# tiborcamargo/KinectPy

Measured on NVIDIA B200. Metric: fused_3kinect_frames_per_s, higher is better.
Workload: dtype f64

## Files before the change

### kinectpy_b200/csrc/kp_batch.cuh

```cuda
#pragma once
#include "kp_common.cuh"
#include "kp_grid.cuh"
#include "kp_vbi.cuh"

struct DCnt {
    const int32_t *p;
    int stride;
#ifdef __CUDACC__
    __device__ __forceinline__ int at(int s) const { return p[(size_t)s * stride]; }
#endif
};
struct DOut {
    int32_t *p;
    int stride;
#ifdef __CUDACC__
    __device__ __forceinline__ int32_t &at(int s) const { return p[(size_t)s * stride]; }
#endif
};
static inline DCnt dcnt(const int32_t *p, size_t stride_bytes) { return DCnt{p, (int)(stride_bytes / 4)}; }
static inline DOut dout(int32_t *p, size_t stride_bytes) { return DOut{p, (int)(stride_bytes / 4)}; }

struct KpVoxDev {
    double minb[3];
    double voxel;
// ... 1 lines not shown
    unsigned int sentinel;
    int imax[3];
    int ok;
};

struct BLaunch {
    kp_ctx *ctx;
    int nseg;
    int64_t cap;
    int ctas;
};

constexpr int BC_THREADS = 256;
constexpr int BC_ITEMS = 8;
constexpr int BC_TILE = BC_THREADS * BC_ITEMS;

struct BScan {
    int32_t *tile_sum;
    unsigned int *ticket;
    int max_tiles;
};

int kp_b_compact_rows(const BLaunch &L, const BScan &S, DCnt n, const uint8_t *mask, int64_t mask_stride, int invert,
                      const float *in, float *out, int64_t row_stride, DOut total, const uint32_t *aux_in = nullptr,
                      uint32_t *aux_out = nullptr);
int kp_b_partition_rows(const BLaunch &L, const BScan &S, DCnt n, const uint8_t *mask, int64_t mask_stride, const float *in,
                        float *out_true, float *out_false, int64_t row_stride, DOut total, const uint32_t *aux_in = nullptr,
                        uint32_t *aux_true = nullptr, uint32_t *aux_false = nullptr);
int kp_b_compact_index(const BLaunch &L, const BScan &S, DCnt n, const uint8_t *mask, int64_t mask_stride, int32_t *list,
                       int64_t list_stride, DOut total);
int kp_b_run_starts_u32(const BLaunch &L, const BScan &S, DCnt n, const uint32_t *keys, int64_t key_stride, int32_t *run_start,
                        int64_t rs_stride, DOut total);
int kp_b_exclusive_scan(const BLaunch &L, const BScan &S, DCnt n, int32_t *v, int64_t v_stride, DOut total);

struct BSort {
    int32_t *g_hist;
    int32_t *g_tot;
};
int kp_b_sort_pairs_u32(const BLaunch &L, const BSort &W, int64_t n, int passes, uint32_t *keys, uint32_t *keys_tmp,
                        int32_t *vals, int32_t *vals_tmp, int64_t stride);
size_t kp_b_sort_hist_elems(int64_t n);

int kp_b_csum(const BLaunch &L, DCnt n, const double *x, int64_t x_stride, int mode, const double *aux, int64_t aux_stride,
              double *tmp, int64_t tmp_stride, double *out, int64_t out_stride);

struct KpKnnSegDesc {
    const KpGridDev *g0, *g1;
    const KpVbiDev *vbi;
    const float4 *pts0;
    const int32_t *n;
    uint8_t *flags0, *flags1;
    int32_t *list0, *list1;
    const int32_t *cnt0, *cnt1;
    const KpGridDev *gm;
    uint8_t *flags_m; int32_t *list_m; const int32_t *cnt_m;
    double *mean;
    const float *cloud;
    float *normals;
};
struct KpKnnBatch {
    void *d_params = nullptr, *h_params = nullptr;
    int nseg = 0, k = 0, mode = 0, cap_hist = 0, cap_warp = 0, rad = 1, cap_mid = 0, has_mid = 0;
};
int kp_knn_batch_create(kp_ctx *ctx, const KpKnnSegDesc *segs, int nseg, int k, int mode, double radius, double rho_a, double rho_b,
                        KpKnnBatch *out);
int kp_knn_batch_vbi(kp_ctx *ctx, const KpKnnBatch &b, int64_t cap_rows);
void kp_knn_batch_destroy(KpKnnBatch *b);
int kp_knn_batch_level0(kp_ctx *ctx, const KpKnnBatch &b, int64_t cap_rows);
int kp_knn_batch_mid(kp_ctx *ctx, const KpKnnBatch &b, int64_t cap_rows);
int kp_knn_batch_level1(kp_ctx *ctx, const KpKnnBatch &b, int64_t cap_rows);
int kp_knn_batch_stragglers(kp_ctx *ctx, const KpKnnBatch &b);

struct KpIcpPairDesc {
    const KpGridDev *tgt_grid;
    const KpVbiDev *tgt_vbi;
    const float *tgt_normals;
    const float *src;
    const int32_t *n_src;
    double init_T[16];
    double *res_T, *res_fit, *res_rmse; int32_t *res_iters;
};
struct KpIcpBatch {
    void *d_params = nullptr, *d_work = nullptr;
    int npairs = 0, max_iter = 0, grid = 0;
    int64_t cap_src = 0;
};
int kp_icp_batch_create(kp_ctx *ctx, const KpIcpPairDesc *pairs, int npairs, int64_t cap_src, double max_corr, int max_iter,
                        double rel_fitness, double rel_rmse, KpIcpBatch *out);
void kp_icp_batch_destroy(KpIcpBatch *b);
int kp_icp_batch_run(kp_ctx *ctx, const KpIcpBatch &b);
```

### kinectpy_b200/csrc/kp_engine.cu

```cuda
#include <stdlib.h>
#include <string.h>
#include <string>
#include <vector>
#include "kp_batch.cuh"

int kp_unproject_engine(kp_ctx *ctx, const uint16_t *d_depth, const float *d_xytab, const double *h_T, int B, int S, int64_t P,
                        int flags, double scale, float *d_xyz, float *d_xyz_raw, int32_t *d_slots, int32_t *d_rows,
                        const uint8_t *d_rgb, const double *d_crop_med, double crop_gate);
size_t kp_unproject_engine_slots(int B, int S, int64_t P);
int kp_crop_median_engine(kp_ctx *ctx, const uint16_t *d_depth, const uint32_t *d_vbits, int B, int S, int64_t P, uint32_t *d_hist,
                          double *d_med);
size_t kp_crop_median_hist_elems();
int kp_resample_engine(kp_ctx *ctx, const float *const *d_base, int64_t stride, const int32_t *d_n, int64_t n_step, int B, int64_t N, int mode,
                       uint64_t seed, const int64_t *h_ids, int32_t *d_status, int64_t status_step, uint32_t *keys, uint32_t *hist,
                       void *st, unsigned long long *list, float *d_out);
size_t kp_resample_engine_hist_elems();
size_t kp_resample_engine_state_bytes();
int64_t kp_resample_engine_cap(int64_t N);
bool kp_resample_engine_fits(int64_t N);

namespace {
constexpr int ENG_MAX_S = 6;
constexpr int ENG_MAX_CAND = 16;

// ... 2041 lines not shown
    return KP_OK;
}

int kp_pipeline_destroy(kp_pipeline *p)
{
    if (!p) return KP_OK;
    cudaSetDevice(p->device);
    for (auto &s : p->slots) slot_destroy(s);
    if (p->d_tab) cudaFree(p->d_tab);
    if (p->d_vbits) cudaFree(p->d_vbits);
    if (p->h_res) cudaFreeHost(p->h_res);
    delete p;
    return KP_OK;
}

const char *kp_pipeline_last_error(kp_pipeline *p) { return p ? p->err.c_str() : kp_last_error(nullptr); }

int kp_pipeline_run(kp_pipeline *p, const uint16_t *depth, int depth_on_device, int64_t F, kp_frame_result *h_results,
                    float *d_out_xyz, int64_t out_stride)
{
    return run_impl(p, depth, nullptr, depth_on_device, F, nullptr, h_results, d_out_xyz, out_stride, nullptr);
}

int kp_pipeline_run_ex(kp_pipeline *p, const uint16_t *depth, const uint8_t *rgb, int inputs_on_device, int64_t F,
                       const int64_t *h_frame_ids, kp_frame_result *h_results, float *d_out_xyz, int64_t out_stride, float *d_fixed)
{
    return run_impl(p, depth, rgb, inputs_on_device, F, h_frame_ids, h_results, d_out_xyz, out_stride, d_fixed);
}

int kp_pipeline_run_host(kp_pipeline *p, const uint16_t *h_depth, int64_t F, kp_frame_result *h_results, float *h_out_xyz,
                         int64_t out_stride)
{
    if (p && h_out_xyz) {
        cudaPointerAttributes at;
        if (cudaPointerGetAttributes(&at, h_out_xyz) != cudaSuccess || (at.type != cudaMemoryTypeHost && at.type != cudaMemoryTypeManaged)) {
            cudaGetLastError();
            p->err = "kp_pipeline_run_host: h_out_xyz must be pinned host memory (kp_host_alloc)";
            return KP_E_ARG;
        }
    }
    return run_impl(p, h_depth, nullptr, 0, F, nullptr, h_results, h_out_xyz, out_stride, nullptr);
}

int64_t kp_pipeline_launch_count(kp_pipeline *p)
{
    int64_t n = 0;
    if (p) {
        n = p->launches;
        for (auto &s : p->slots) n += s.ctx->launches + s.aux->launches;
    }
    return n;
}

int kp_pipeline_frames_in_flight(kp_pipeline *p, int *batch, int *slots)
{
    if (!p) return KP_E_ARG;
    if (batch) *batch = p->B;
    if (slots) *slots = p->W;
    return KP_OK;
}

int kp_pipeline_frame_counts(kp_pipeline *p, int64_t *h_counts, int n)
{
    if (!p || !h_counts || n < 26) return KP_E_ARG;
    cudaSetDevice(p->device);
    EngSlot &s = p->slots[0];
    if (cudaStreamSynchronize(s.ctx->stream) != cudaSuccess) return KP_E_CUDA;
    EngDyn d;
    if (cudaMemcpy(&d, s.dyn, sizeof d, cudaMemcpyDeviceToHost) != cudaSuccess) return KP_E_CUDA;
    std::vector<EngCloud> cl((size_t)p->cfg.S);
    if (cudaMemcpy(cl.data(), s.icl, sizeof(EngCloud) * cl.size(), cudaMemcpyDeviceToHost) != cudaSuccess) return KP_E_CUDA;
    const int64_t v[8] = {d.n_fused, d.n_voxel, d.n_sor, d.n_lo, d.n_rest, d.n_merged, d.n_fsor, d.n_out};
    for (int i = 0; i < 8; ++i) h_counts[i] = v[i];
    for (int i = 0; i < 3; ++i) { h_counts[8 + i] = d.cnt_l0[i]; h_counts[11 + i] = d.cnt_l1[i]; }
    for (int i = 0; i < 6; ++i) { h_counts[14 + i] = i < p->cfg.S ? cl[i].nv : 0; h_counts[20 + i] = i < p->cfg.S ? cl[i].n : 0; }
    if (n >= 29)
        for (int i = 0; i < 3; ++i) h_counts[26 + i] = d.cnt_lm[i];
    if (n >= 35) {
        double med[ENG_MAX_S] = {0.0};
        if (p->cfg.do_crop && cudaMemcpy(med, s.crop_med, sizeof(double) * p->cfg.S, cudaMemcpyDeviceToHost) != cudaSuccess) return KP_E_CUDA;
        for (int i = 0; i < 6; ++i) h_counts[29 + i] = i < p->cfg.S ? (int64_t)(2.0 * med[i]) : 0;
    }
    if (n >= 36) h_counts[35] = p->cfg.ror_nb_points > 0 ? d.n_ror : 0;
    return KP_OK;
}

int kp_pipeline_profile(kp_pipeline *p, int enable_or_read, int max_entries, const char **h_names, double *h_ms,
                        int64_t *h_calls, double *h_bytes, int *h_n)
{
    if (!p) return KP_E_ARG;
    cudaSetDevice(p->device);
    kp_ctx *ctx = p->slots[0].ctx;
    if (enable_or_read == 1 || enable_or_read == 0) {
        kp_profile_reset(ctx);
        kp_profile_enable(ctx, enable_or_read);
        p->profiling = enable_or_read == 1;
        return KP_OK;
    }
    return kp_profile_read(ctx, max_entries, h_names, h_ms, h_calls, h_bytes, h_n);
}

}
```

### kinectpy_b200/csrc/kp_icp.cu

```cuda
#include <math.h>
#include <string.h>
#include <stdlib.h>
#include <vector>
#include "kp_grid.cuh"
#include "kp_batch.cuh"
#include "kp_umeyama.cuh"

namespace {
#ifndef ICP_THREADS_N
#define ICP_THREADS_N 256
#endif
constexpr int ICP_THREADS = ICP_THREADS_N;
#ifndef ICP_MIN_CTAS
#define ICP_MIN_CTAS 4
#endif
constexpr int ICP_GROUP = 32;
constexpr int ICP_NV = 29;
enum { ICP_PLANE = 0, ICP_POINT = 1, ICP_COLORED = 2 };

struct IcpState {
    double T[16];
    double U[16];
    double fitness, rmse;
    long long ncorr;
    int done, iters;
    unsigned int ticket;
    int pass;
    double slack;
};

struct IcpParams {
    KpGridDev g;
    const float *tgt_normals;
    int mode;
    const float *src_int;
    const float *tgt_int;
    const float *tgt_grad;
    double sqrt_lg, sqrt_lp;
    double *cur;
    int32_t *corr;
    int ns;
    double r2;
    double slack;
    int max_iter;
    double rel_fit, rel_rmse;
    IcpState *st;
    double *slots;
    double *gslots;
    unsigned int *gticket;
    const KpGridDev *gdev;
    const int32_t *ns_dev;
    const float *src;
    double max_corr;
    double init_T[16];
    double *res_T, *res_fit, *res_rmse; int32_t *res_iters;
    const KpVbiDev *vbi;
};

__device__ __forceinline__ double icp_slack(const KpGridDev &g, double max_corr)
{
    double M = 0.0;
    for (int c = 0; c < 3; ++c)
        M = fmax(M, fmax(fabs(g.org[c]), fabs(g.org[c] + g.cell * (double)g.dim[c])) + 2.0 * max_corr);
    const double eps = 8.0 * M / 16777216.0;
    return eps * (2.0 * max_corr + eps) * 1.000001 + 4e-6 * (max_corr * max_corr);
}

__device__ __forceinline__ IcpParams icp_params_batched(const IcpParams *__restrict__ pp)
{
    IcpParams p = pp[blockIdx.y];
    p.g = *p.gdev;
    p.ns = *p.ns_dev;
    p.slack = p.st->slack;
    return p;
}

__global__ void __launch_bounds__(256) k_icp_init(const float *src, int ns, const __grid_constant__ IcpParams p, IcpState init,
                                                  double *out)
{
    int i = blockIdx.x * blockDim.x + threadIdx.x;
    if (i == 0) *p.st = init;
    if (i >= ns) return;
    const double *T = init.T;
    double X = src[3 * (int64_t)i], Y = src[3 * (int64_t)i + 1], Z = src[3 * (int64_t)i + 2];
    out[3 * (int64_t)i] = kp_affine(T[0], T[1], T[2], T[3], X, Y, Z);
    out[3 * (int64_t)i + 1] = kp_affine(T[4], T[5], T[6], T[7], X, Y, Z);
    out[3 * (int64_t)i + 2] = kp_affine(T[8], T[9], T[10], T[11], X, Y, Z);
}

__device__ __forceinline__ int icp_nearest(const KpGridDev &g, double sx, double sy, double sz, double r2, double slack, int prev)
{
    int bpos = -1;
    const int cx = kp_cell_coord(g, sx, 0), cy = kp_cell_coord(g, sy, 1), cz = kp_cell_coord(g, sz, 2);
    double bd = INFINITY;
    int bi = -1;
    const float fx32 = (float)sx, fy32 = (float)sy, fz32 = (float)sz;
    if (prev >= 0) {
        const float4 q = __ldg(g.pts + prev);
        const double d2 = kp_d2(sx, sy, sz, (double)q.x, (double)q.y, (double)q.z);
        if (d2 < r2) { bd = d2; bi = __float_as_int(q.w); bpos = prev; }
    }
    float flo[3], fhi[3];
    {
        const double cs = g.cell * (1.0 - 3.0 / 1048576.0);
        const double ss[3] = {sx, sy, sz};
        const int cc[3] = {cx, cy, cz};
#pragma unroll
        for (int c = 0; c < 3; ++c) {
            const double f = fmin(fmax((ss[c] - g.org[c]) * g.inv_cell - (double)cc[c], 0.0), 1.0);
            flo[c] = (float)(f * cs); fhi[c] = (float)((1.0 - f) * cs);
        }
    }
    const double lim0 = fmin(bd, r2);
    const float budget = __double2float_ru(lim0 * (1.0 + 4e-6));
    int2 rng[9];
#pragma unroll
    for (int oi = 0; oi < 9; ++oi) {
        const int dx = oi / 3 - 1, dy = oi % 3 - 1;
        const float gx = dx < 0 ? flo[0] : (dx > 0 ? fhi[0] : 0.0f), gy = dy < 0 ? flo[1] : (dy > 0 ? fhi[1] : 0.0f);
        const float zb = budget - (gx * gx + gy * gy);
        const int zlo = flo[2] * flo[2] <= zb ? cz - 1 : cz, zhi = fhi[2] * fhi[2] <= zb ? cz + 1 : cz;
        rng[oi] = zb >= 0.0f ? kp_span_range(g, cx + dx, cy + dy, zlo, zhi) : make_int2(0, 0);
    }
    float lim32 = __double2float_ru(lim0 + slack), cur = budget;
    const int order[9] = {4, 1, 3, 5, 7, 0, 2, 6, 8};
#pragma unroll
    for (int k = 0; k < 9; ++k) {
        const int oi = order[k], dx = oi / 3 - 1, dy = oi % 3 - 1;
        const float gx = dx < 0 ? flo[0] : (dx > 0 ? fhi[0] : 0.0f), gy = dy < 0 ? flo[1] : (dy > 0 ? fhi[1] : 0.0f);
        if (gx * gx + gy * gy > cur) continue;
        for (int t = rng[oi].x; t < rng[oi].y; t += 4) {
            const int m = rng[oi].y - t;
            float4 q[4];
            q[0] = __ldg(g.pts + t);
            q[1] = __ldg(g.pts + (m > 1 ? t + 1 : t));
            q[2] = __ldg(g.pts + (m > 2 ? t + 2 : t));
            q[3] = __ldg(g.pts + (m > 3 ? t + 3 : t));
            float d32[4];
#pragma unroll
            for (int u = 0; u < 4; ++u) {
                const float ex = fx32 - q[u].x, ey = fy32 - q[u].y, ez = fz32 - q[u].z;
                d32[u] = __fmaf_rn(ez, ez, __fmaf_rn(ey, ey, ex * ex));
            }
#pragma unroll
            for (int u = 0; u < 4; ++u) {
                if (u >= m || d32[u] > lim32) continue;
                const double d2 = kp_d2(sx, sy, sz, (double)q[u].x, (double)q[u].y, (double)q[u].z);
                const int id = __float_as_int(q[u].w);
                if (d2 < r2 && (d2 < bd || (d2 == bd && id < bi))) {
                    bd = d2; bi = id; bpos = t + u;
                    lim32 = __double2float_ru(bd + slack); cur = __double2float_ru(bd * (1.0 + 4e-6));
                }
            }
        }
    }
    return bpos;
}

__device__ __forceinline__ int icp_nearest_vbi(const KpVbiDev &v, double sx, double sy, double sz, double r2, double slack, int prev)
{
    int bpos = -1, bi = -1;
    double bd = INFINITY;
    if (prev >= 0) {
        const float4 q = __ldg(v.pts + prev);
        const double d2 = kp_d2(sx, sy, sz, (double)q.x, (double)q.y, (double)q.z);
        if (d2 < r2) { bd = d2; bi = __float_as_int(q.w); bpos = prev; }
    }
    const double lim0 = fmin(bd, r2);
    const double rad = sqrt(lim0) * (1.0 + 1e-6) + v.eps + v.voxel * 1e-6;
    KpVbiBox box;
    if (!kp_vbi_box(v, sx, sy, sz, rad, box)) return bpos;
    const float fx32 = (float)sx, fy32 = (float)sy, fz32 = (float)sz;
    float lim32 = __double2float_ru(lim0 + slack);
    kp_vbi_visit(v, box, [&](int pos, const float4 &q) {
        const float ex = fx32 - q.x, ey = fy32 - q.y, ez = fz32 - q.z;
        const float d32 = __fmaf_rn(ez, ez, __fmaf_rn(ey, ey, ex * ex));
        if (d32 > lim32) return;
        const double d2 = kp_d2(sx, sy, sz, (double)q.x, (double)q.y, (double)q.z);
        const int id = __float_as_int(q.w);
        if (d2 < r2 && (d2 < bd || (d2 == bd && id < bi))) {
            bd = d2; bi = id; bpos = pos;
            lim32 = __double2float_ru(bd + slack);
        }
    });
    return bpos;
}

__device__ bool icp_solve6_cta(double (*M)[7], double *x, int tid)
{
    const int r = tid / 7, j = tid % 7;
    const bool own = tid < 42;
    bool ok = true;
    for (int c = 0; c < 6; ++c) {
        int pv = c;
        double best = fabs(M[c][c]);
        for (int rr = c + 1; rr < 6; ++rr) {
            const double v = fabs(M[rr][c]);
            if (v > best) { best = v; pv = rr; }
        }
        if (!(best > 1e-300)) { ok = false; break; }
        __syncthreads();
        if (own && r == c && pv != c) { const double t = M[c][j]; M[c][j] = M[pv][j]; M[pv][j] = t; }
        __syncthreads();
        double nv = 0.0;
        const bool upd = own && r > c && j >= c;
        if (upd) { const double f = M[r][c] / M[c][c]; nv = M[r][j] - f * M[c][j]; }
        __syncthreads();
        if (upd) M[r][j] = nv;
        __syncthreads();
    }
    if (ok && tid == 0) {
        for (int rr = 5; rr >= 0; --rr) {
            double sacc = M[rr][6];
            for (int jj = rr + 1; jj < 6; ++jj) sacc -= M[rr][jj] * x[jj];
            x[rr] = sacc / M[rr][rr];
        }
    }
    __syncthreads();
    if (ok)
        for (int rr = 0; rr < 6; ++rr) if (!isfinite(x[rr])) ok = false;
    return ok;
}

__device__ void icp_finish(const IcpParams &p, IcpState *st, const double *tot, int pass, int tid)
{
    __shared__ double M[6][7];
    __shared__ double x[6];
    __shared__ double Un[16];
    __shared__ int s_done;
    const double nc = tot[28];
    if (tid == 0) {
        const double fit = p.ns > 0 ? nc / (double)p.ns : 0.0;
        const double rmse = nc > 0 ? sqrt(tot[27] / nc) : 0.0;
        const double pfit = st->fitness, prmse = st->rmse;
        st->fitness = fit; st->rmse = rmse; st->ncorr = (long long)nc;
        st->ticket = 0;
        st->pass = pass + 1;
        bool done = false;
        if (pass > 0) {
            st->iters = pass;
            if (fabs(pfit - fit) < p.rel_fit && fabs(prmse - rmse) < p.rel_rmse) done = true;
        }
        if (pass >= p.max_iter) done = true;
        if (done) st->done = 1;
        s_done = done ? 1 : 0;
    }
    if (tid < 16) Un[tid] = (tid % 5 == 0) ? 1.0 : 0.0;
    if (tid < 6) x[tid] = 0.0;
    __syncthreads();
    if (s_done) return;
    if (p.mode == ICP_POINT) {
        if (tid == 0 && nc > 0) kp_umeyama(tot, nc, Un);
    } else {
        if (tid < 42) {
            const int r = tid / 7, j = tid % 7;
            if (j == 6) M[r][6] = -tot[21 + r];
            else {
                const int a = r < j ? r : j, b = r < j ? j : r;
                M[r][j] = tot[a * 6 - (a * (a - 1)) / 2 + (b - a)];
            }
        }
        __syncthreads();
        const bool ok = icp_solve6_cta(M, x, tid);
        if (ok && nc > 0 && tid == 0) {
            double ca = cos(x[0]), sa = sin(x[0]), cb = cos(x[1]), sb = sin(x[1]), cg = cos(x[2]), sg = sin(x[2]);
            Un[0] = cg * cb; Un[1] = cg * sb * sa - sg * ca; Un[2] = cg * sb * ca + sg * sa; Un[3] = x[3];
            Un[4] = sg * cb; Un[5] = sg * sb * sa + cg * ca; Un[6] = sg * sb * ca - cg * sa; Un[7] = x[4];
            Un[8] = -sb;     Un[9] = cb * sa;                Un[10] = cb * ca;               Un[11] = x[5];
        }
    }
    __syncthreads();
    double tn = 0.0;
    if (tid < 16) {
        const int i2 = tid >> 2, j = tid & 3;
        for (int k = 0; k < 4; ++k) tn = tn + Un[4 * i2 + k] * st->T[4 * k + j];
    }
    __syncthreads();
    if (tid < 16) { st->T[tid] = tn; st->U[tid] = Un[tid]; }
    __threadfence();
}

template <int MODE>
__device__ __forceinline__ void icp_iter_body(const IcpParams &p)
{
    __shared__ double sh[ICP_THREADS / 32][ICP_NV];
    __shared__ double part[ICP_THREADS / 32][32];
    __shared__ double tot[ICP_NV];
    __shared__ unsigned int s_ticket;
    IcpState *st = p.st;
    const int tid = threadIdx.x, lane = tid & 31, warp = tid >> 5;
    const int i = blockIdx.x * ICP_THREADS + tid;
    double sx0 = 0.0, sy0 = 0.0, sz0 = 0.0;
    int prev0 = -1;
    if (i < p.ns) {
        sx0 = p.cur[3 * (int64_t)i]; sy0 = p.cur[3 * (int64_t)i + 1]; sz0 = p.cur[3 * (int64_t)i + 2];
        prev0 = p.corr[i];
    }
    if (st->done) return;
    const int pass = st->pass;
    const KpGridDev &g = p.g;
    bool has = false;
    double J[6] = {0, 0, 0, 0, 0, 0}, r = 0.0, bd = 0.0;
    double J2[6] = {0, 0, 0, 0, 0, 0}, r2v = 0.0;
    if (i < p.ns) {
        double sx = sx0, sy = sy0, sz = sz0;
        int prev = pass > 0 ? prev0 : -1;
        if (pass > 0) {
            const double *U = st->U;
            const double x2 = kp_affine(U[0], U[1], U[2], U[3], sx, sy, sz);
            const double y2 = kp_affine(U[4], U[5], U[6], U[7], sx, sy, sz);
            const double z2 = kp_affine(U[8], U[9], U[10], U[11], sx, sy, sz);
            sx = x2; sy = y2; sz = z2;
            p.cur[3 * (int64_t)i] = sx; p.cur[3 * (int64_t)i + 1] = sy; p.cur[3 * (int64_t)i + 2] = sz;
        }
        int bpos = -1;
        const bool use_vbi = p.vbi != nullptr && p.vbi->ok;
        if (use_vbi) {
            if (!isnan(sx)) { const KpVbiDev v = *p.vbi; bpos = icp_nearest_vbi(v, sx, sy, sz, p.r2, p.slack, prev); }
        } else if (!isnan(sx) && g.dim[0] > 0) bpos = icp_nearest(g, sx, sy, sz, p.r2, p.slack, prev);
        p.corr[i] = bpos;
        if (bpos >= 0) {
            has = true;
            const float4 q = __ldg((use_vbi ? p.vbi->pts : g.pts) + bpos);
            const int bi = __float_as_int(q.w);
            const double ex = sx - (double)q.x, ey = sy - (double)q.y, ez = sz - (double)q.z;
            bd = (ex * ex + ey * ey) + ez * ez;
            if (MODE == ICP_POINT) {
                J[0] = sx; J[1] = sy; J[2] = sz; J[3] = (double)q.x; J[4] = (double)q.y; J[5] = (double)q.z;
            } else {
                const double nx = (double)__ldg(p.tgt_normals + 3 * (int64_t)bi), ny = (double)__ldg(p.tgt_normals + 3 * (int64_t)bi + 1),
                             nz = (double)__ldg(p.tgt_normals + 3 * (int64_t)bi + 2);
                r = (ex * nx + ey * ny) + ez * nz;
                J[0] = sy * nz - sz * ny; J[1] = sz * nx - sx * nz; J[2] = sx * ny - sy * nx; J[3] = nx; J[4] = ny; J[5] = nz;
                if (MODE == ICP_COLORED) {
                    const double is = (double)__ldg(p.src_int + i), it = (double)__ldg(p.tgt_int + bi);
                    const double gx = (double)__ldg(p.tgt_grad + 3 * (int64_t)bi), gy = (double)__ldg(p.tgt_grad + 3 * (int64_t)bi + 1),
                                 gz = (double)__ldg(p.tgt_grad + 3 * (int64_t)bi + 2);
                    const double px = ex - r * nx, py = ey - r * ny, pz = ez - r * nz;
                    const double is_proj = ((gx * px + gy * py) + gz * pz) + it;
                    const double gn = (gx * nx + gy * ny) + gz * nz;
                    const double mx = -(gx - gn * nx), my = -(gy - gn * ny), mz = -(gz - gn * nz);
                    J2[0] = p.sqrt_lp * (sy * mz - sz * my); J2[1] = p.sqrt_lp * (sz * mx - sx * mz); J2[2] = p.sqrt_lp * (sx * my - sy * mx);
                    J2[3] = p.sqrt_lp * mx; J2[4] = p.sqrt_lp * my; J2[5] = p.sqrt_lp * mz;
                    r2v = p.sqrt_lp * (is - is_proj);
#pragma unroll
                    for (int a = 0; a < 6; ++a) J[a] *= p.sqrt_lg;
                    r *= p.sqrt_lg;
                }
            }
        }
    }
    if (__any_sync(KP_FULL, has)) {
        double v[32];
        if (MODE == ICP_POINT) {
#pragma unroll
            for (int a = 0; a < 6; ++a) v[a] = J[a];
#pragma unroll
            for (int a = 0; a < 3; ++a)
#pragma unroll
                for (int b = 0; b < 3; ++b) v[6 + 3 * a + b] = J[3 + a] * J[b];
#pragma unroll
            for (int a = 15; a < 27; ++a) v[a] = 0.0;
        } else {
            int k = 0;
#pragma unroll
            for (int a = 0; a < 6; ++a)
#pragma unroll
                for (int b = a; b < 6; ++b) { v[k] = J[a] * J[b]; if (MODE == ICP_COLORED) v[k] += J2[a] * J2[b]; ++k; }
#pragma unroll
            for (int a = 0; a < 6; ++a) { v[21 + a] = J[a] * r; if (MODE == ICP_COLORED) v[21 + a] += J2[a] * r2v; }
        }
        v[27] = bd; v[28] = has ? 1.0 : 0.0; v[29] = 0.0; v[30] = 0.0; v[31] = 0.0;
#pragma unroll
        for (int s = 16; s >= 1; s >>= 1) {
            const bool upper = (lane & s) != 0;
#pragma unroll
            for (int j = 0; j < s; ++j) {
                const double send = upper ? v[j] : v[j + s];
                const double keep = upper ? v[j + s] : v[j];
                v[j] = keep + __shfl_xor_sync(KP_FULL, send, s);
            }
        }
        if (lane < ICP_NV) sh[warp][lane] = v[0];
    } else if (lane < ICP_NV) {
        sh[warp][lane] = 0.0;
    }
    __syncthreads();
    if (tid < ICP_NV) {
        double s = 0;
        for (int w = 0; w < ICP_THREADS / 32; ++w) s += sh[w][tid];
        p.slots[(size_t)blockIdx.x * ICP_NV + tid] = s;
    }
    constexpr int W = ICP_THREADS / 32;
    const unsigned nact = max(1u, ((unsigned)p.ns + ICP_THREADS - 1) / ICP_THREADS);
    const unsigned group = blockIdx.x / ICP_GROUP, ngroups = (nact + ICP_GROUP - 1) / ICP_GROUP;
    const unsigned g0 = group * ICP_GROUP, gsize = min((unsigned)ICP_GROUP, nact - g0);
    auto fold = [&](const double *rows, unsigned nrows, double *dst_sh) {
        double sacc = 0;
        if (lane < ICP_NV) {
            unsigned r = warp;
            for (; r + 3 * W < nrows; r += 4 * W) {
                double t[4];
#pragma unroll
                for (int u = 0; u < 4; ++u) t[u] = __ldcg(rows + (size_t)(r + u * W) * ICP_NV + lane);
#pragma unroll
                for (int u = 0; u < 4; ++u) sacc += t[u];
            }
            for (; r < nrows; r += W) sacc += __ldcg(rows + (size_t)r * ICP_NV + lane);
        }
        part[warp][lane] = sacc;
        __syncthreads();
        if (tid < ICP_NV) {
            double t = 0;
            for (int w = 0; w < W; ++w) t += part[w][tid];
            dst_sh[tid] = t;
        }
        __syncthreads();
    };
    __threadfence();
    __syncthreads();
    if (tid == 0) s_ticket = atomicAdd(&p.gticket[group], 1u);
    __syncthreads();
    if (s_ticket != gsize - 1) return;
    __threadfence();
    fold(p.slots + (size_t)g0 * ICP_NV, gsize, tot);
    if (tid < ICP_NV) p.gslots[(size_t)group * ICP_NV + tid] = tot[tid];
    if (tid == 0) p.gticket[group] = 0;
    __threadfence();
    __syncthreads();
    if (tid == 0) s_ticket = atomicAdd(&st->ticket, 1u);
    __syncthreads();
    if (s_ticket != ngroups - 1) return;
    __threadfence();
    fold(p.gslots, ngroups, tot);
    __syncthreads();
    icp_finish(p, st, tot, pass, tid);
}
template <int MODE>
__global__ void __launch_bounds__(ICP_THREADS, ICP_MIN_CTAS) k_icp_iter(const __grid_constant__ IcpParams p)
{
    icp_iter_body<MODE>(p);
}
#ifndef ICP_B_CTAS
#define ICP_B_CTAS 3
#endif
template <int MODE>
__global__ void __launch_bounds__(ICP_THREADS, ICP_B_CTAS) k_icp_iter_b(const IcpParams *pp)
{
    const IcpParams *me = pp + blockIdx.y;
    const int ns = *me->ns_dev;
    if (blockIdx.x * ICP_THREADS >= (unsigned)max(ns, 1) || me->st->done) return;
    const IcpParams p = icp_params_batched(pp);
    icp_iter_body<MODE>(p);
}
__global__ void __launch_bounds__(256) k_icp_init_b(const IcpParams *pp)
{
    const IcpParams *p = pp + blockIdx.y;
    const int ns = *p->ns_dev;
    if (blockIdx.x == 0 && threadIdx.x == 0) {
        IcpState init;
        memset(&init, 0, sizeof init);
        for (int i = 0; i < 16; ++i) { init.T[i] = p->init_T[i]; init.U[i] = (i % 5 == 0) ? 1.0 : 0.0; }
        if (p->vbi && p->vbi->ok) {
            const KpVbiDev &v = *p->vbi;
            double M = 0.0;
            for (int c = 0; c < 3; ++c)
                M = fmax(M, fmax(fabs(v.minb[c]), fabs(v.minb[c] + v.voxel * (double)v.nvox[c])) + 2.0 * p->max_corr);
            const double eps = 8.0 * M / 16777216.0;
            init.slack = eps * (2.0 * p->max_corr + eps) * 1.000001 + 4e-6 * (p->max_corr * p->max_corr);
        } else init.slack = icp_slack(*p->gdev, p->max_corr);
        *p->st = init;
    }
    const double *T = p->init_T;
    for (int i = blockIdx.x * blockDim.x + threadIdx.x; i < ns; i += gridDim.x * blockDim.x) {
        const double X = p->src[3 * (int64_t)i], Y = p->src[3 * (int64_t)i + 1], Z = p->src[3 * (int64_t)i + 2];
        p->cur[3 * (int64_t)i] = kp_affine(T[0], T[1], T[2], T[3], X, Y, Z);
        p->cur[3 * (int64_t)i + 1] = kp_affine(T[4], T[5], T[6], T[7], X, Y, Z);
        p->cur[3 * (int64_t)i + 2] = kp_affine(T[8], T[9], T[10], T[11], X, Y, Z);
    }
}
__global__ void k_icp_results_b(const IcpParams *pp, int npairs)
{
    const int i = blockIdx.x * blockDim.x + threadIdx.x;
    if (i >= npairs) return;
    const IcpParams &p = pp[i];
    const IcpState *st = p.st;
    for (int e = 0; e < 16; ++e) p.res_T[e] = st->T[e];
    *p.res_fit = st->fitness; *p.res_rmse = st->rmse; *p.res_iters = st->iters;
}
}

int kp_icp_batch_create(kp_ctx *ctx, const KpIcpPairDesc *pairs, int npairs, int64_t cap_src, double max_corr, int max_iter,
                        double rel_fitness, double rel_rmse, KpIcpBatch *out)
{
    out->npairs = npairs; out->max_iter = max_iter < 0 ? 0 : max_iter; out->cap_src = cap_src;
    const int grid = (int)kp_blocks(cap_src > 0 ? cap_src : 1, ICP_THREADS);
    const int ngroups = (grid + ICP_GROUP - 1) / ICP_GROUP;
    out->grid = grid;
    const size_t per_pair = (size_t)cap_src * 3 * sizeof(double) + (size_t)cap_src * sizeof(int32_t) + (size_t)grid * ICP_NV * sizeof(double) +
                            (size_t)ngroups * ICP_NV * sizeof(double) + (size_t)ngroups * sizeof(unsigned int) + sizeof(IcpState) + 1024;
    KP_CUDA(ctx, cudaMalloc(&out->d_work, per_pair * (size_t)npairs));
    KP_CUDA(ctx, cudaMemset(out->d_work, 0, per_pair * (size_t)npairs));
    std::vector<IcpParams> h((size_t)npairs);
    char *w = (char *)out->d_work;
    auto take = [&](size_t bytes) { char *r = w; w += (bytes + 255) & ~(size_t)255; return r; };
    for (int i = 0; i < npairs; ++i) {
        IcpParams p;
        memset(&p, 0, sizeof p);
        p.tgt_normals = pairs[i].tgt_normals; p.mode = ICP_PLANE;
        p.sqrt_lg = 1.0; p.sqrt_lp = 0.0;
        p.cur = (double *)take((size_t)cap_src * 3 * sizeof(double));
        p.corr = (int32_t *)take((size_t)cap_src * sizeof(int32_t));
        p.slots = (double *)take((size_t)grid * ICP_NV * sizeof(double));
        p.gslots = (double *)take((size_t)ngroups * ICP_NV * sizeof(double));
        p.gticket = (unsigned int *)take((size_t)ngroups * sizeof(unsigned int));
        p.st = (IcpState *)take(sizeof(IcpState));
        p.r2 = max_corr * max_corr; p.max_corr = max_corr;
        p.max_iter = out->max_iter; p.rel_fit = rel_fitness; p.rel_rmse = rel_rmse;
        p.gdev = pairs[i].tgt_grid; p.ns_dev = pairs[i].n_src; p.src = pairs[i].src; p.vbi = pairs[i].tgt_vbi;
        for (int e = 0; e < 16; ++e) p.init_T[e] = pairs[i].init_T[e];
        p.res_T = pairs[i].res_T; p.res_fit = pairs[i].res_fit; p.res_rmse = pairs[i].res_rmse; p.res_iters = pairs[i].res_iters;
        h[i] = p;
    }
    KP_CUDA(ctx, cudaMalloc(&out->d_params, sizeof(IcpParams) * h.size()));
    KP_CUDA(ctx, cudaMemcpy(out->d_params, h.data(), sizeof(IcpParams) * h.size(), cudaMemcpyHostToDevice));
    return KP_OK;
}
void kp_icp_batch_destroy(KpIcpBatch *b)
{
    if (!b) return;
    if (b->d_params) cudaFree(b->d_params);
    if (b->d_work) cudaFree(b->d_work);
    b->d_params = b->d_work = nullptr;
}
int kp_icp_batch_run(kp_ctx *ctx, const KpIcpBatch &b)
{
    KpProfScope prof_scope__(ctx, "icp");
    const IcpParams *pp = (const IcpParams *)b.d_params;
    int64_t gi = (b.cap_src + 255) / 256;
    if (gi > (int64_t)ctx->sm_count * 8) gi = (int64_t)ctx->sm_count * 8;
    k_icp_init_b<<<dim3((unsigned)(gi > 0 ? gi : 1), (unsigned)b.npairs), 256, 0, ctx->stream>>>(pp);
    KP_LAUNCH_CHECK(ctx);
    for (int i = 0; i <= b.max_iter; ++i) {
        k_icp_iter_b<ICP_PLANE><<<dim3((unsigned)b.grid, (unsigned)b.npairs), ICP_THREADS, 0, ctx->stream>>>(pp);
        KP_LAUNCH_CHECK(ctx);
    }
    k_icp_results_b<<<kp_blocks(b.npairs, 64), 64, 0, ctx->stream>>>(pp, b.npairs);
    KP_LAUNCH_CHECK(ctx);
    return KP_OK;
}


namespace {
__global__ void __launch_bounds__(256) k_intensity(const float *colors, int64_t n, const int32_t *order, float *out)
{
    int64_t i = (int64_t)blockIdx.x * blockDim.x + threadIdx.x;
    if (i >= n) return;
    const int64_t j = order ? order[i] : i;
    out[i] = (float)((((double)colors[3 * j] + (double)colors[3 * j + 1]) + (double)colors[3 * j + 2]) / 3.0);
}

__global__ void __launch_bounds__(128) k_color_gradient(const float *xyz, const float *inten, const float *nrm, int64_t n,
                                                        const int32_t *idx, const int32_t *cnt, int k, float *grad)
{
    int64_t i = (int64_t)blockIdx.x * blockDim.x + threadIdx.x;
    if (i >= n) return;
    const int nn = cnt[i];
    double x[3] = {0, 0, 0};
    if (nn >= 4 && !isnan(xyz[3 * i])) {
        const double vx = xyz[3 * i], vy = xyz[3 * i + 1], vz = xyz[3 * i + 2];
        const double nx = nrm[3 * i], ny = nrm[3 * i + 1], nz = nrm[3 * i + 2];
        const double it = inten[i];
        double A[6] = {0, 0, 0, 0, 0, 0}, b[3] = {0, 0, 0};
        for (int t = 1; t < nn; ++t) {
            const int64_t j = idx[i * k + t];
            const double ax = (double)xyz[3 * j] - vx, ay = (double)xyz[3 * j + 1] - vy, az = (double)xyz[3 * j + 2] - vz;
            const double dn = (ax * nx + ay * ny) + az * nz;
            const double px = ax - dn * nx, py = ay - dn * ny, pz = az - dn * nz;
            const double di = (double)inten[j] - it;
            A[0] += px * px; A[1] += px * py; A[2] += px * pz; A[3] += py * py; A[4] += py * pz; A[5] += pz * pz;
            b[0] += px * di; b[1] += py * di; b[2] += pz * di;
        }
        const double w = (double)(nn - 1);
        A[0] += w * nx * w * nx; A[1] += w * nx * w * ny; A[2] += w * nx * w * nz;
        A[3] += w * ny * w * ny; A[4] += w * ny * w * nz; A[5] += w * nz * w * nz;
        double M[3][4] = {{A[0], A[1], A[2], b[0]}, {A[1], A[3], A[4], b[1]}, {A[2], A[4], A[5], b[2]}};
        bool ok = true;
        for (int c = 0; c < 3 && ok; ++c) {
            int pv = c;
            for (int r2 = c + 1; r2 < 3; ++r2) if (fabs(M[r2][c]) > fabs(M[pv][c])) pv = r2;
            if (!(fabs(M[pv][c]) > 1e-300)) { ok = false; break; }
            if (pv != c) for (int j = 0; j < 4; ++j) { const double tv = M[c][j]; M[c][j] = M[pv][j]; M[pv][j] = tv; }
            for (int r2 = c + 1; r2 < 3; ++r2) { const double f = M[r2][c] / M[c][c]; for (int j = c; j < 4; ++j) M[r2][j] -= f * M[c][j]; }
        }
        if (ok) {
            x[2] = M[2][3] / M[2][2];
            x[1] = (M[1][3] - M[1][2] * x[2]) / M[1][1];
            x[0] = (M[0][3] - M[0][1] * x[1] - M[0][2] * x[2]) / M[0][0];
            if (!(isfinite(x[0]) && isfinite(x[1]) && isfinite(x[2]))) x[0] = x[1] = x[2] = 0.0;
        }
    }
    grad[3 * i] = (float)x[0]; grad[3 * i + 1] = (float)x[1]; grad[3 * i + 2] = (float)x[2];
}
}

int kp_color_gradient_device(kp_ctx *ctx, const float *d_xyz, const float *d_colors, const float *d_normals, int64_t n,
                             double radius, int max_nn, float *d_intensity, float *d_grad)
{
    if (n <= 0) return KP_OK;
    if (max_nn < 1 || !(radius > 0.0)) return kp_set_err(ctx, KP_E_ARG, "colour gradient: radius <= 0 or max_nn < 1");
    k_intensity<<<kp_blocks(n, 256), 256, 0, ctx->stream>>>(d_colors, n, nullptr, d_intensity);
    KP_LAUNCH_CHECK(ctx);
    KpGrid g;
    KP_TRY(kp_grid_build_knn(ctx, d_xyz, n, radius * (1.0 + 4e-6), max_nn, nullptr, &g));
    int32_t *idx, *cnt;
    KP_TRY(kp_ws(ctx, (size_t)n * (size_t)max_nn, &idx));
    KP_TRY(kp_ws(ctx, (size_t)n, &cnt));
    KP_TRY(kp_knn_device(ctx, g, nullptr, n, max_nn, radius, idx, nullptr, cnt, nullptr, d_xyz));
    KP_PROFB(ctx, "color_gradient", (double)n * (4.0 * max_nn + 12.0 + 12.0 + 4.0 + 12.0));
    k_color_gradient<<<kp_blocks(n, 128), 128, 0, ctx->stream>>>(d_xyz, d_intensity, d_normals, n, idx, cnt, max_nn, d_grad);
    KP_LAUNCH_CHECK(ctx);
    return KP_OK;
}

int kp_icp_device(kp_ctx *ctx, const float *d_src, int64_t n_src, const KpGrid &tgt_grid, const float *d_tgt_normals,
                  double max_corr, const double *h_init16, int max_iter, double rel_fitness, double rel_rmse,
                  double *h_T_out, double *h_fitness, double *h_rmse, int *h_iters, int64_t *h_ncorr, const KpIcpExtra *extra)
{
// ... 142 lines not shown
```

### kinectpy_b200/pipeline.py

```python
from __future__ import annotations

import ctypes as C
from dataclasses import dataclass, field
from typing import List, Optional

import numpy as np

from . import _cabi
from ._cabi import FrameResult, KinectPyB200Error, PipelineCfg


@dataclass
class PipelineConfig:
    n_sensors: int = 3
    pixels: int = 1024 * 1024
    unproject_flags: int = _cabi.UNPROJECT_INT16 | _cabi.UNPROJECT_DROP_ANY_ZERO
    scale: float = 1e-3
    voxel_size: float = 0.01
    sor_k: int = 20
    sor_ratio: float = 2.0
    do_floor: bool = True
    floor_band: float = 0.20
    ransac_thr: float = 0.01
    ransac_n: int = 3
# ... 91 lines not shown
    def upload(self, depth: np.ndarray, rgb: Optional[np.ndarray] = None):
        d = self._ctx.to_device(depth, np.uint16)
        if rgb is None:
            self._ctx.sync()
            return d
        r = self._ctx.to_device(rgb, np.uint8)
        self._ctx.sync()
        return d, r

    def run(self, depth, rgb=None, n_frames: Optional[int] = None, want_points: bool = False, out_stride: Optional[int] = None,
            want_fixed: bool = False, frame_ids=None, check: bool = True):
        S, P = self.cfg.n_sensors, self.cfg.pixels
        on_dev = isinstance(depth, _cabi.DeviceArray)
        if on_dev:
            F = int(depth.shape[0]) if n_frames is None else int(n_frames)
            ptr = depth.ptr
            rptr = rgb.ptr if rgb is not None else None
        else:
            depth = np.ascontiguousarray(depth, dtype=np.uint16).reshape(-1, S, P)
            F = depth.shape[0] if n_frames is None else int(n_frames)
            ptr = depth.ctypes.data
            if rgb is not None:
                rgb = np.ascontiguousarray(rgb, dtype=np.uint8).reshape(-1, S, P, 3)
            rptr = rgb.ctypes.data if rgb is not None else None
        res = (FrameResult * F)()
        out = None
        stride = 0
        if want_points:
            stride = int(out_stride or S * P)
            out = self._ctx.empty((F, stride, 3), np.float32)
            self._ctx.sync()
        fixed = None
        if want_fixed:
            fixed = self._ctx.empty((F, max(int(self.cfg.resample_n), 1), 3), np.float32)
            self._ctx.sync()
        ids = None
        if frame_ids is not None:
            ids = np.ascontiguousarray(frame_ids, dtype=np.int64).reshape(-1)
            if ids.size != F:
                raise ValueError("frame_ids must hold one id per frame")
        rc = self.lib.kp_pipeline_run_ex(self.handle, ptr, rptr, 1 if on_dev else 0, F, ids.ctypes.data if ids is not None else None,
                                         res, out.ptr if out is not None else None, stride, fixed.ptr if fixed is not None else None)
        if rc != 0 and (check or all(res[f].status == 0 for f in range(F))):
            self._raise(rc)
        outs: List[FrameOutput] = []
        host = out.to_host() if out is not None else None
        hfixed = fixed.to_host() if fixed is not None else None
        for f in range(F):
            r = res[f]
            T = np.array([list(r.icp_T[i]) for i in range(max(S - 1, 0))], dtype=np.float64).reshape(-1, 4, 4)
            fo = FrameOutput(r.n_fused, r.n_voxel, r.n_sor, r.n_floor_inliers, r.n_out, T,
                             np.array(list(r.icp_fitness)[:S - 1]), np.array(list(r.icp_rmse)[:S - 1]),
                             np.array(list(r.icp_iters)[:S - 1]))
            fo.status = int(r.status)
            fo.floor_plane = np.array(list(r.floor_plane), dtype=np.float64)
            if host is not None:
                fo.points = host[f, :r.n_out].copy()
            if hfixed is not None:
                fo.fixed = hfixed[f].copy()
            outs.append(fo)
        self._last_raw = res
        return outs

    def run_raw(self, depth_ptr: int, on_device: bool, n_frames: int, d_out_ptr=None, out_stride: int = 0):
        res = (FrameResult * n_frames)()
        rc = self.lib.kp_pipeline_run(self.handle, depth_ptr, 1 if on_device else 0, n_frames, res, d_out_ptr, out_stride)
        if rc != 0:
            self._raise(rc)
        return res

    def run_host(self, h_depth_ptr: int, n_frames: int, h_out_ptr: int, out_stride: int):
        res = (FrameResult * n_frames)()
        rc = self.lib.kp_pipeline_run_host(self.handle, h_depth_ptr, n_frames, res, h_out_ptr, out_stride)
        if rc != 0:
            self._raise(rc)
        return res

    def frames_in_flight(self):
        b, w = C.c_int(), C.c_int()
        self.lib.kp_pipeline_frames_in_flight(self.handle, C.byref(b), C.byref(w))
        return b.value, w.value

    def frame_counts(self) -> dict:
        v = (C.c_int64 * 36)()
        rc = self.lib.kp_pipeline_frame_counts(self.handle, v, 36)
        if rc != 0:
            self._raise(rc)
        S = self.cfg.n_sensors
        d = dict(zip(("n_fused", "n_voxel", "n_sor", "n_lo", "n_rest", "n_merged", "n_fsor", "n_out"), [int(x) for x in v[:8]]))
        d["n_inl"] = d["n_lo"] - d["n_rest"]
        d["leftovers_l0"], d["leftovers_l1"] = [int(x) for x in v[8:11]], [int(x) for x in v[11:14]]
        d["leftovers_mid"] = [int(x) for x in v[26:29]]
        d["nv_icp"], d["n_icp"] = [int(x) for x in v[14:14 + S]], [int(x) for x in v[20:20 + S]]
        d["crop_median"] = [int(x) / 2.0 for x in v[29:29 + S]]
        d["n_ror"] = int(v[35])
        return d

    def launch_count(self) -> int:
        return int(self.lib.kp_pipeline_launch_count(self.handle))

    def profile(self, on: bool):
        rc = self.lib.kp_pipeline_profile(self.handle, 1 if on else 0, 0, None, None, None, None, None)
        if rc != 0:
            self._raise(rc)

    def profile_read(self):
        names = (C.c_char_p * 64)()
        ms = (C.c_double * 64)()
        calls = (C.c_int64 * 64)()
        by = (C.c_double * 64)()
        n = C.c_int()
        rc = self.lib.kp_pipeline_profile(self.handle, 2, 64, names, ms, calls, by, C.byref(n))
        if rc != 0:
            self._raise(rc)
        return {names[i].decode(): {"ms": float(ms[i]), "calls": int(calls[i]), "bytes": float(by[i])} for i in range(n.value)}
```

Measured before the change: 189.4.

## Replace fixed ICP iteration launches with a graph while-loop that exits on convergence

When the stream is being captured into a CUDA graph, the fixed max_iter+1 launches of the batched ICP iteration kernel become a conditional while node. An atomic counter of converged pairs clears the loop condition once every pair is done. This removes the leftover launches that previously ran only to return early after convergence. It needs CUDA 12.4+ conditional-node support, adds per-pass atomics, and adds a pass counter exposed through frame_counts.

```diff
diff --git a/kinectpy_b200/csrc/kp_batch.cuh b/kinectpy_b200/csrc/kp_batch.cuh
--- a/kinectpy_b200/csrc/kp_batch.cuh
+++ b/kinectpy_b200/csrc/kp_batch.cuh
@@ -107,6 +107,8 @@
 };
 struct KpIcpBatch {
     void *d_params = nullptr, *d_work = nullptr;
+    unsigned int *d_ndone = nullptr;
+    unsigned int *d_passes = nullptr;
     int npairs = 0, max_iter = 0, grid = 0;
     int64_t cap_src = 0;
 };
diff --git a/kinectpy_b200/csrc/kp_engine.cu b/kinectpy_b200/csrc/kp_engine.cu
--- a/kinectpy_b200/csrc/kp_engine.cu
+++ b/kinectpy_b200/csrc/kp_engine.cu
@@ -2147,6 +2147,11 @@
         for (int i = 0; i < 6; ++i) h_counts[29 + i] = i < p->cfg.S ? (int64_t)(2.0 * med[i]) : 0;
     }
     if (n >= 36) h_counts[35] = p->cfg.ror_nb_points > 0 ? d.n_ror : 0;
+    if (n >= 37) {
+        unsigned int passes = 0;
+        if (s.icp.d_passes && cudaMemcpy(&passes, s.icp.d_passes, sizeof passes, cudaMemcpyDeviceToHost) != cudaSuccess) return KP_E_CUDA;
+        h_counts[36] = passes;
+    }
     return KP_OK;
 }
 
diff --git a/kinectpy_b200/csrc/kp_icp.cu b/kinectpy_b200/csrc/kp_icp.cu
--- a/kinectpy_b200/csrc/kp_icp.cu
+++ b/kinectpy_b200/csrc/kp_icp.cu
@@ -57,6 +57,13 @@
     const KpVbiDev *vbi;
 };
 
+struct IcpLoop {
+    unsigned int *ndone;
+    unsigned int npairs;
+    cudaGraphConditionalHandle h;
+    unsigned int *passes;
+};
+
 __device__ __forceinline__ double icp_slack(const KpGridDev &g, double max_corr)
 {
     double M = 0.0;
@@ -222,7 +229,7 @@
     return ok;
 }
 
-__device__ void icp_finish(const IcpParams &p, IcpState *st, const double *tot, int pass, int tid)
+__device__ void icp_finish(const IcpParams &p, IcpState *st, const double *tot, int pass, int tid, const IcpLoop &loop)
 {
     __shared__ double M[6][7];
     __shared__ double x[6];
@@ -242,7 +249,10 @@
             if (fabs(pfit - fit) < p.rel_fit && fabs(prmse - rmse) < p.rel_rmse) done = true;
         }
         if (pass >= p.max_iter) done = true;
-        if (done) st->done = 1;
+        if (done) {
+            st->done = 1;
+            if (loop.ndone && atomicAdd(loop.ndone, 1u) + 1u == loop.npairs) cudaGraphSetConditional(loop.h, 0);
+        }
         s_done = done ? 1 : 0;
     }
     if (tid < 16) Un[tid] = (tid % 5 == 0) ? 1.0 : 0.0;
@@ -281,7 +291,7 @@
 }
 
 template <int MODE>
-__device__ __forceinline__ void icp_iter_body(const IcpParams &p)
+__device__ __forceinline__ void icp_iter_body(const IcpParams &p, const IcpLoop &loop)
 {
     __shared__ double sh[ICP_THREADS / 32][ICP_NV];
     __shared__ double part[ICP_THREADS / 32][32];
@@ -434,29 +444,31 @@
     __threadfence();
     fold(p.gslots, ngroups, tot);
     __syncthreads();
-    icp_finish(p, st, tot, pass, tid);
+    icp_finish(p, st, tot, pass, tid, loop);
 }
 template <int MODE>
 __global__ void __launch_bounds__(ICP_THREADS, ICP_MIN_CTAS) k_icp_iter(const __grid_constant__ IcpParams p)
 {
-    icp_iter_body<MODE>(p);
+    icp_iter_body<MODE>(p, IcpLoop{nullptr, 0u, 0, nullptr});
 }
 #ifndef ICP_B_CTAS
 #define ICP_B_CTAS 3
 #endif
 template <int MODE>
-__global__ void __launch_bounds__(ICP_THREADS, ICP_B_CTAS) k_icp_iter_b(const IcpParams *pp)
+__global__ void __launch_bounds__(ICP_THREADS, ICP_B_CTAS) k_icp_iter_b(const IcpParams *pp, const __grid_constant__ IcpLoop loop)
 {
     const IcpParams *me = pp + blockIdx.y;
     const int ns = *me->ns_dev;
+    if (blockIdx.x == 0 && blockIdx.y == 0 && threadIdx.x == 0) ++*loop.passes;
     if (blockIdx.x * ICP_THREADS >= (unsigned)max(ns, 1) || me->st->done) return;
     const IcpParams p = icp_params_batched(pp);
-    icp_iter_body<MODE>(p);
-}
-__global__ void __launch_bounds__(256) k_icp_init_b(const IcpParams *pp)
+    icp_iter_body<MODE>(p, loop);
+}
+__global__ void __launch_bounds__(256) k_icp_init_b(const IcpParams *pp, unsigned int *ndone, unsigned int *passes)
 {
     const IcpParams *p = pp + blockIdx.y;
     const int ns = *p->ns_dev;
+    if (blockIdx.x == 0 && blockIdx.y == 0 && threadIdx.x == 0) { *ndone = 0; *passes = 0; }
     if (blockIdx.x == 0 && threadIdx.x == 0) {
         IcpState init;
         memset(&init, 0, sizeof init);
@@ -499,11 +511,13 @@
     out->grid = grid;
     const size_t per_pair = (size_t)cap_src * 3 * sizeof(double) + (size_t)cap_src * sizeof(int32_t) + (size_t)grid * ICP_NV * sizeof(double) +
                             (size_t)ngroups * ICP_NV * sizeof(double) + (size_t)ngroups * sizeof(unsigned int) + sizeof(IcpState) + 1024;
-    KP_CUDA(ctx, cudaMalloc(&out->d_work, per_pair * (size_t)npairs));
-    KP_CUDA(ctx, cudaMemset(out->d_work, 0, per_pair * (size_t)npairs));
+    KP_CUDA(ctx, cudaMalloc(&out->d_work, 256 + per_pair * (size_t)npairs));
+    KP_CUDA(ctx, cudaMemset(out->d_work, 0, 256 + per_pair * (size_t)npairs));
     std::vector<IcpParams> h((size_t)npairs);
     char *w = (char *)out->d_work;
     auto take = [&](size_t bytes) { char *r = w; w += (bytes + 255) & ~(size_t)255; return r; };
+    out->d_ndone = (unsigned int *)take(2 * sizeof(unsigned int));
+    out->d_passes = out->d_ndone + 1;
     for (int i = 0; i < npairs; ++i) {
         IcpParams p;
         memset(&p, 0, sizeof p);
@@ -532,6 +546,7 @@
     if (b->d_params) cudaFree(b->d_params);
     if (b->d_work) cudaFree(b->d_work);
     b->d_params = b->d_work = nullptr;
+    b->d_ndone = b->d_passes = nullptr;
 }
 int kp_icp_batch_run(kp_ctx *ctx, const KpIcpBatch &b)
 {
@@ -539,11 +554,34 @@
     const IcpParams *pp = (const IcpParams *)b.d_params;
     int64_t gi = (b.cap_src + 255) / 256;
     if (gi > (int64_t)ctx->sm_count * 8) gi = (int64_t)ctx->sm_count * 8;
-    k_icp_init_b<<<dim3((unsigned)(gi > 0 ? gi : 1), (unsigned)b.npairs), 256, 0, ctx->stream>>>(pp);
+    k_icp_init_b<<<dim3((unsigned)(gi > 0 ? gi : 1), (unsigned)b.npairs), 256, 0, ctx->stream>>>(pp, b.d_ndone, b.d_passes);
     KP_LAUNCH_CHECK(ctx);
-    for (int i = 0; i <= b.max_iter; ++i) {
-        k_icp_iter_b<ICP_PLANE><<<dim3((unsigned)b.grid, (unsigned)b.npairs), ICP_THREADS, 0, ctx->stream>>>(pp);
-        KP_LAUNCH_CHECK(ctx);
+    const dim3 grid((unsigned)b.grid, (unsigned)b.npairs);
+    cudaStreamCaptureStatus cs = cudaStreamCaptureStatusNone;
+    cudaGraph_t cg = nullptr;
+    const cudaGraphNode_t *deps = nullptr;
+    size_t ndeps = 0;
+    KP_CUDA(ctx, cudaStreamGetCaptureInfo(ctx->stream, &cs, nullptr, &cg, &deps, &ndeps));
+    if (cs == cudaStreamCaptureStatusActive) {
+        cudaGraphConditionalHandle h;
+        KP_CUDA(ctx, cudaGraphConditionalHandleCreate(&h, cg, 1, cudaGraphCondAssignDefault));
+        cudaGraphNodeParams cp = {cudaGraphNodeTypeConditional};
+        cp.conditional.handle = h; cp.conditional.type = cudaGraphCondTypeWhile; cp.conditional.size = 1;
+        cudaGraphNode_t loop_node, pass_node;
+        KP_CUDA(ctx, cudaGraphAddNode(&loop_node, cg, deps, ndeps, &cp));
+        IcpLoop loop{b.d_ndone, (unsigned)b.npairs, h, b.d_passes};
+        void *args[] = {(void *)&pp, (void *)&loop};
+        cudaKernelNodeParams kp;
+        memset(&kp, 0, sizeof kp);
+        kp.func = (void *)k_icp_iter_b<ICP_PLANE>; kp.gridDim = grid; kp.blockDim = dim3(ICP_THREADS); kp.kernelParams = args;
+        KP_CUDA(ctx, cudaGraphAddKernelNode(&pass_node, cp.conditional.phGraph_out[0], nullptr, 0, &kp));
+        KP_CUDA(ctx, cudaStreamUpdateCaptureDependencies(ctx->stream, &loop_node, 1, cudaStreamSetCaptureDependencies));
+        ctx->launches++;
+    } else {
+        for (int i = 0; i <= b.max_iter; ++i) {
+            k_icp_iter_b<ICP_PLANE><<<grid, ICP_THREADS, 0, ctx->stream>>>(pp, IcpLoop{nullptr, 0u, 0, b.d_passes});
+            KP_LAUNCH_CHECK(ctx);
+        }
     }
     k_icp_results_b<<<kp_blocks(b.npairs, 64), 64, 0, ctx->stream>>>(pp, b.npairs);
     KP_LAUNCH_CHECK(ctx);
diff --git a/kinectpy_b200/pipeline.py b/kinectpy_b200/pipeline.py
--- a/kinectpy_b200/pipeline.py
+++ b/kinectpy_b200/pipeline.py
@@ -197,8 +197,8 @@
         return b.value, w.value
 
     def frame_counts(self) -> dict:
-        v = (C.c_int64 * 36)()
-        rc = self.lib.kp_pipeline_frame_counts(self.handle, v, 36)
+        v = (C.c_int64 * 37)()
+        rc = self.lib.kp_pipeline_frame_counts(self.handle, v, 37)
         if rc != 0:
             self._raise(rc)
         S = self.cfg.n_sensors
@@ -209,6 +209,7 @@
         d["nv_icp"], d["n_icp"] = [int(x) for x in v[14:14 + S]], [int(x) for x in v[20:20 + S]]
         d["crop_median"] = [int(x) / 2.0 for x in v[29:29 + S]]
         d["n_ror"] = int(v[35])
+        d["icp_passes"] = int(v[36])
         return d
 
     def launch_count(self) -> int:
```

New measurement: 194.0 (median of 6 runs). 2.4% higher.
